# libav/libav

Measured on AMD Instinct MI355X. Metric: macroblocks_per_s, higher is better.
Workload: dtype u8

## Files before the change

include/mi355_h264_frame.h:

```cpp
#ifndef MI355_H264_FRAME_H
#define MI355_H264_FRAME_H

#include <stddef.h>
#include <stdint.h>

#ifdef __cplusplus
extern "C" {
#endif

#define MI355_MB_INTRA4x4    0x00000001u
#define MI355_MB_INTRA16x16  0x00000002u
#define MI355_MB_INTRA_PCM   0x00000004u
#define MI355_MB_16x16       0x00000008u
#define MI355_MB_16x8        0x00000010u
#define MI355_MB_8x16        0x00000020u
#define MI355_MB_8x8         0x00000040u
#define MI355_MB_P0L0        0x00001000u
#define MI355_MB_P1L0        0x00002000u
#define MI355_MB_P0L1        0x00004000u
#define MI355_MB_P1L1        0x00008000u
#define MI355_MB_8x8DCT      0x01000000u
#define MI355_MB_INTRA       (MI355_MB_INTRA4x4 | MI355_MB_INTRA16x16 | MI355_MB_INTRA_PCM)

#define MI355_MBF_LEFT_EDGE  0x01
#define MI355_MBF_TOP_EDGE   0x02
#define MI355_MBF_NO_DEBLOCK 0x04
#define MI355_MBF_WEIGHTED   0x08
#define MI355_MBF_BYPASS     0x10
#define MI355_MBF_BYPASS_PRED 0x20
#define MI355_MBF_BYPASS_X264OLD 0x40
#define MI355_MBF_FILTER_OWN_SLICE 0x80

#define MI355_SUB_8x8  0
#define MI355_SUB_8x4  1
#define MI355_SUB_4x8  2
#define MI355_SUB_4x4  3
#define MI355_SUB_L0   0x10
#define MI355_SUB_L1   0x20

#define MI355_NNZ_LUMA(i)   (i)
#define MI355_NNZ_CB(j)     (16 + (j))
#define MI355_NNZ_CR(j)     (20 + (j))
#define MI355_NNZ_LUMA_DC   24
#define MI355_NNZ_CB_DC     25
#define MI355_NNZ_CR_DC     26

typedef struct mi355_h264_mb {
    uint32_t mb_type;
    uint32_t nnz_mask;
    uint16_t cbp;
    int8_t   qp;
    uint8_t  flags;
    int8_t   slice_alpha_c0_offset;
    int8_t   slice_beta_offset;
    uint8_t  intra16x16_pred_mode;
    uint8_t  chroma_pred_mode;
    uint16_t topleft_samples_available;
    uint16_t topright_samples_available;
    uint8_t  sub_mb_type[4];
    int8_t   ref_idx[2][4];
    uint32_t dc_qmul[3];
    uint8_t  slice_id;
    uint8_t  intra_level;
    uint8_t  qpc[2];
    union {
        int8_t intra4x4_pred_mode[16];
        struct {
            uint8_t ref_pic[2][4];
            int8_t  chroma_dy[2][4];
        } inter;
    } u;
} mi355_h264_mb;

#define MI355_H264_COEFS_PER_MB 384
static inline int mi355_luma_dc_slot(int k)
{
    static const uint8_t col[4] = { 0, 2, 8, 10 }, row[4] = { 0, 1, 4, 5 };
    return 16 * (col[k >> 2] + row[k & 3]);
}


#define MI355_H264_MAX_REFS 16
#define MI355_H264_MAX_SLOTS 32

typedef struct mi355_h264_slice {
    uint8_t use_weight;
    uint8_t use_weight_chroma;
    uint8_t luma_log2_weight_denom;
    uint8_t chroma_log2_weight_denom;
    uint8_t list_count;
    uint8_t reserved[3];
    uint8_t ref_slot[2][MI355_H264_MAX_REFS];
    int16_t luma_weight[MI355_H264_MAX_REFS][2][2];
    int16_t chroma_weight[MI355_H264_MAX_REFS][2][2][2];
    int16_t implicit_weight[MI355_H264_MAX_REFS][MI355_H264_MAX_REFS];
    uint8_t chroma_qp_table[2][52];
    int16_t implicit_weight_field[2][2 * MI355_H264_MAX_REFS][2 * MI355_H264_MAX_REFS];
} mi355_h264_slice;

typedef struct mi355_h264_frame {
    int32_t mb_width, mb_height;
    uint8_t *dst[3];
    int32_t dst_stride[2];
    uint8_t *recon[3];
    int32_t recon_stride[2];
    const uint8_t *ref[MI355_H264_MAX_SLOTS][3];
    const mi355_h264_mb *mb;
    const int16_t *mv[2];
    const int16_t *coef;
    const mi355_h264_slice *slices;
    int32_t nslices;
    int32_t max_intra_level;
    const uint32_t *intra_list;
    const int32_t *intra_level_start;
    int32_t max_level_width;
    int32_t field_picture;
    int32_t surface_layout;
    int32_t flags;
} mi355_h264_frame;
#define MI355_FRAME_NO_INTER 1
#define MI355_FRAME_MBAFF    2

#define MI355_SURFACE_LINEAR 0
#define MI355_SURFACE_TILED  1
#define MI355_LAYOUTS_LINEAR 1
#define MI355_LAYOUTS_TILED  2
#define MI355_TILE_LUMA_BYTES   256
#define MI355_TILE_CHROMA_BYTES 128

typedef struct mi355_surface_job {
    uint8_t *lin[3];
    uint8_t *tiled[2];
    int32_t lin_stride[2];
    int32_t tiled_stride[2];
    int32_t mb_width, mb_height;
    int32_t to_tiled;
    int32_t reserved0;
} mi355_surface_job;
int mi355_h264_surface_convert_dev(const mi355_surface_job *jobs, int n, int max_mb_width, int max_mb_height, void *stream);

int mi355_h264_decode_frames(const mi355_h264_frame *frames, int nframes, void *stream);

int mi355_h264_decode_frames_dev(const mi355_h264_frame *d_frames, int nframes,
                                 int max_mb_width, int max_mb_height, int max_intra_level,
                                 int max_level_width, void *stream);

int mi355_h264_decode_frames_levels_dev(const mi355_h264_frame *d_frames, int nframes,
                                        int max_mb_width, int max_mb_height, int max_intra_level,
                                        const int32_t *level_widths, void *stream);

int mi355_h264_decode_frames_layouts_dev(const mi355_h264_frame *d_frames, int nframes,
                                         int max_mb_width, int max_mb_height, int max_intra_level,
                                         const int32_t *level_widths, int layouts, void *stream);

int mi355_h264_decode_frames_wide_dev(const mi355_h264_frame *d_frames, int nframes, int max_mb_width, int max_mb_height,
                                      int max_intra_level, const int32_t *level_widths, int bit_depth, int chroma_format_idc,
                                      int passes, void *stream);

int mi355_h264_recon_intra_levels_dev(const mi355_h264_frame *d_frames, int nframes, int max_intra_level, const int32_t *level_widths, void *stream);
int mi355_h264_recon_intra_all_dev(const mi355_h264_frame *d_frames, int nframes, int max_mb_width, int max_mb_height, int max_intra_level, const int32_t *level_widths, void *stream);
int mi355_h264_recon_intra_plan(int max_mb_width, int max_mb_height, int max_intra_level, const int32_t *level_widths, int pinned, int *single, long long *per_picture);
int mi355_h264_recon_inter_dev(const mi355_h264_frame *d_frames, int nframes, int max_mb_width, int max_mb_height, void *stream);
int mi355_h264_recon_inter_layouts_dev(const mi355_h264_frame *d_frames, int nframes, int max_mb_width, int max_mb_height, int layouts, void *stream);
int mi355_h264_recon_run_plan(int nframes, int max_mb_width, int max_mb_height, int forced, int *run, int *runs_row);
int mi355_h264_recon_inter_run_dev(const mi355_h264_frame *d_frames, int nframes, int max_mb_width, int max_mb_height, int run, void *stream);
int mi355_h264_recon_inter_sparse_dev(const mi355_h264_frame *d_frames, int nframes, int max_mb_width, int max_mb_height, void *stream);
int mi355_h264_recon_intra_dev(const mi355_h264_frame *d_frames, int nframes, int max_intra_level, int max_level_width, void *stream);
int mi355_h264_deblock_dev(const mi355_h264_frame *d_frames, int nframes, int max_mb_width, int max_mb_height, void *stream);
int mi355_h264_deblock_layouts_dev(const mi355_h264_frame *d_frames, int nframes, int max_mb_width, int max_mb_height, int layouts, void *stream);

typedef struct mi355_h264_deblock_plan_info {
    int32_t tiled_waves;
    int32_t linear_bands;
    int32_t skip_tiled;
    int32_t linear_launches;
} mi355_h264_deblock_plan_info;
int mi355_h264_deblock_plan(int nframes, int max_mb_width, int max_mb_height, int layouts, int cus, mi355_h264_deblock_plan_info *plan);
int mi355_h264_deblock_form_dev(const mi355_h264_frame *d_frames, int nframes, int max_mb_width, int max_mb_height, int layouts,
                                int tiled_waves, int linear_bands, void *stream);

int mi355_h264_intra_schedule(mi355_h264_mb *mb, int mb_width, int mb_height,
                              uint32_t *list, int32_t *level_start, int *max_level_width);

int mi355_h264_intra_schedule_mbaff(mi355_h264_mb *mb, int mb_width, int mb_height,
                                    uint32_t *list, int32_t *level_start, int *max_level_width);

void *mi355_malloc(size_t bytes);
void  mi355_free(void *dptr);
int   mi355_memcpy_h2d(void *dst, const void *src, size_t bytes);
int   mi355_memcpy_d2h(void *dst, const void *src, size_t bytes);
int   mi355_memcpy_d2d(void *dst, const void *src, size_t bytes);
int   mi355_sync(void *stream);
void  mi355_prefer_blocking_sync(int on);
void *mi355_host_alloc(size_t bytes);
void  mi355_host_free(void *p);
int   mi355_memcpy_h2d_async(void *dst, const void *src, size_t bytes, void *stream);
int   mi355_memcpy_d2h_async(void *dst, const void *src, size_t bytes, void *stream);
int   mi355_memcpy2d_d2h_async(void *dst, size_t dst_pitch, const void *src, size_t src_pitch, size_t width_bytes, size_t rows, void *stream);
int   mi355_memcpy2d_d2d_async(void *dst, size_t dst_pitch, const void *src, size_t src_pitch, size_t width_bytes, size_t rows, void *stream);
int   mi355_event_sync(void *event);
typedef struct mi355_copy_job {
    const void *src;
    void *dst;
    uint64_t bytes;
} mi355_copy_job;
int   mi355_copy_batch_dev(const mi355_copy_job *jobs, int n, size_t max_bytes, void *stream);
typedef struct mi355_h264_pipelines mi355_h264_pipelines;
mi355_h264_pipelines *mi355_h264_pipelines_create(int shares, int turns);
void mi355_h264_pipelines_destroy(mi355_h264_pipelines *p);
int  mi355_h264_pipelines_decode_dev(mi355_h264_pipelines *p, const mi355_h264_frame *d_frames, int nframes, int max_mb_width, int max_mb_height,
                                     int max_intra_level, const int32_t *level_widths, int layouts);
int  mi355_h264_pipelines_sync(mi355_h264_pipelines *p);
int  mi355_h264_pipelines_share(const mi355_h264_pipelines *p, int nframes, int share, int *first, int *count);
void mi355_h264_pipelines_timing(mi355_h264_pipelines *p, int on);
void mi355_h264_pipelines_join(mi355_h264_pipelines *p, int mode);
int  mi355_h264_pipelines_collect(mi355_h264_pipelines *p, double sums[3], int *launches);

void *mi355_stream_create(void);
void  mi355_stream_destroy(void *stream);
int   mi355_stream_wait_event(void *stream, void *event);
void *mi355_event_create(void);
void  mi355_event_destroy(void *event);
int   mi355_event_record(void *event, void *stream);
int   mi355_event_query(void *event);
float mi355_event_elapsed_ms(void *start, void *end);

#ifdef __cplusplus
}
#endif
#endif
```

libav_amd/csrc/h264_deblock.hip:

```cpp
#include <cstdlib>
#include <vector>
#include "h264_deblock_dev.h"

using namespace mi355;

namespace {

#ifdef MI355_PROF
__device__ unsigned long long g_prof[16];
#define PROF_MARK(i) do { const unsigned long long now_ = __builtin_readcyclecounter(); prof_acc[i] += now_ - prof_t; prof_t = now_; } while (0)
#else
#define PROF_MARK(i) do { } while (0)
#endif

#ifndef MI355_DCH_LOG
#define MI355_DCH_LOG 2
#endif
constexpr int DCH_LOG = MI355_DCH_LOG, DCH = 1 << DCH_LOG;
#ifndef MI355_DPAD
#define MI355_DPAD 8
#endif
constexpr int DY_PITCH = 16 * DCH + MI355_DPAD;
constexpr int DC_PITCH = 8 * DCH + MI355_DPAD;
constexpr int DIO_ROWS = 16 / DCH;
// ... 543 lines not shown
        if (lane < 52) {
            s.t_alpha[lane] = k_alpha[lane]; s.t_beta[lane] = k_beta[lane];
            s.t_tc0[lane] = ((uint32_t)k_tc0[lane][0] << 8) | ((uint32_t)k_tc0[lane][1] << 16) | ((uint32_t)k_tc0[lane][2] << 24);
        }
        if (lane < 16) {
            const int seg = l >> 2, edge = l & 3, qe = edge == 0 ? 3 : edge - 1;
            const bool outer = edge == 0;
            uint32_t *r = s.role[l];
            r[0] = 1u << blk_index(edge, seg); r[1] = 1u << blk_index(qe, seg); r[2] = 8u * ((edge >> 1) + 2 * (seg >> 1)); r[3] = 8u * ((qe >> 1) + 2 * (seg >> 1));
            r[4] = 1u << blk_index(seg, edge); r[5] = 1u << blk_index(seg, qe); r[6] = 8u * ((seg >> 1) + 2 * (edge >> 1)); r[7] = 8u * ((seg >> 1) + 2 * (qe >> 1));
            r[8] = (uint32_t)(4 * (edge + 4 * seg));
            r[9] = (uint32_t)(outer ? 4 * (3 + 4 * seg) - 64 : 4 * (edge - 1 + 4 * seg));
            r[10] = (uint32_t)(4 * (seg + 4 * edge));
            r[11] = (uint32_t)(outer ? 4 * (seg + 12) - 64 * W : 4 * (seg + 4 * (edge - 1)));
        }
    }
    if (NW == 1) MI355_WAVE_SYNC(); else MI355_WG_BARRIER_LDS();

    uint8_t *const lds = reinterpret_cast<uint8_t *>(&s);
    constexpr uint32_t OY = (uint32_t)offsetof(Deblock3Lds, y), OC = (uint32_t)offsetof(Deblock3Lds, c), OA = (uint32_t)offsetof(Deblock3Lds, above);
    uint32_t k_g2, k_rec, k_topd, k_dy, k_dc, k_gc2, k_da, k_sab, k_sc, k_sd, k_se, k_la, k_lc, k_ld, k_rv, k_cv, k_flags;
    uint32_t k_pl, k_pc, k_hy, k_ha, k_hc, k_hca;
    enum { KF_ROW = 1, KF_TOP = 2, KF_BOTTOM = 4, KF_LO = 8, KF_G0 = 16, KF_ROW0 = 32, KF_CSRC_SHIFT = 8, KF_EDGE8_SHIFT = 16 };
    constexpr uint32_t OP = (uint32_t)offsetof(Deblock3Lds, parm), PB = (uint32_t)sizeof(uint32_t[4][9][2]);
    {
        const int lane = lane_id(), g = lane >> 4, l = lane & 15, ga = (g - 1) & 3;
        const int mb_y = 4 * band + g, mb_yc = mb_y < H ? mb_y : H - 1;
        const bool row_ok = mb_y < H, has_t = row_ok && mb_y > 0, bottom = row_ok && (g == 3 || mb_y == H - 1), lo = l < 8;
        k_flags = (row_ok ? KF_ROW : 0) | (has_t ? KF_TOP : 0) | (bottom ? KF_BOTTOM : 0) | (lo ? KF_LO : 0) | (g == 0 ? KF_G0 : 0) | (mb_yc == 0 ? KF_ROW0 : 0);
        k_flags |= (uint32_t)(4 * ((lane & ~15) | (((l & 7) >> 1) << 2))) << KF_CSRC_SHIFT;
        k_flags |= (uint32_t)(8 * (l & 3)) << KF_EDGE8_SHIFT;
        k_g2 = (uint32_t)(2 * g);
        k_rec = (uint32_t)(64 * mb_yc * W);
        k_topd = mb_yc > 0 ? 64u * (uint32_t)W : 0u;
        k_dy = (uint32_t)(mb_yc * rs + 16 * (l ^ g));
        {
            const int gc = (lane >> 3) & 3, q = lane & 7, yc = 4 * band + gc < H ? 4 * band + gc : H - 1;
            k_dc = (uint32_t)(yc * rcs + 16 * (q ^ gc));
            k_gc2 = (uint32_t)(2 * gc);
        }
        k_da = (lane & 8) ? (uint32_t)(ya * dcs + 16 * ((lane & 7) ^ 3)) : (uint32_t)(ya * ds + 128 + 16 * ((lane & 7) ^ 3));
        k_sab = lo ? (uint32_t)(mb_y * ds - (2 * g + 1) * 256 + 16 * l) : (uint32_t)((mb_y - 1) * ds - 2 * g * 256 + 16 * l);
        k_sc = (uint32_t)((mb_y - 1) * dcs - 2 * g * 128 + 8 * l);
        k_sd = (uint32_t)(mb_y * ds - (2 * g + 1) * 256 + 128 + 8 * l);
        k_se = (uint32_t)(mb_y * dcs - (2 * g + 1) * 128 + 8 * l);
        k_rv = (uint32_t)(256 * g + 16 * (l ^ g));
        k_cv = (uint32_t)(128 * g + 16 * ((l >> 1) ^ g) + 8 * (l & 1));
        k_la = lo ? k_rv : (uint32_t)(g ? 256 * ga + 128 + 16 * ((l - 8) ^ ga) : 16 * ((l - 8) ^ 3));
        k_lc = (uint32_t)(g ? 128 * ga + 16 * ((l >> 1) ^ ga) + 8 * (l & 1) : 128 + 16 * ((l >> 1) ^ 3) + 8 * (l & 1));
        k_ld = (uint32_t)(256 * g + 16 * ((8 + (l >> 1)) ^ g) + 8 * (l & 1));
        k_pl = OP + (uint32_t)(72 * g);
        k_pc = k_pl + (uint32_t)(24 + 24 * (l >> 3));
        k_hy = (uint32_t)(256 * g + 16 * g + l);
        k_ha = (uint32_t)(g ? 256 * ga + 128 + 64 + 16 * ga + l : 64 + 16 * 3 + l);
        k_hc = (uint32_t)(128 * g + 16 * g + 64 * (l >> 3) + (l & 7));
        k_hca = (uint32_t)(g ? 128 * ga + 16 * (ga ^ 3) + 64 * (l >> 3) + (l & 7) : 128 + 64 * (l >> 3) + (l & 7));
        static_assert((OY & 63) == 0 && (OC & 63) == 0 && (OA & 63) == 0, "bits 4 and 5 of a column's address are the swizzle's alone");
    }
    auto kf = [&](uint32_t bit) { return (k_flags & bit) != 0; };
    auto prefetch = [&](Pre &p, int t1) {
        const int l = lane_id() & 15;
        const bool outer = (l & 3) == 0;
        const int xc = med3i(t1 - (int)k_g2, 0, W - 1);
        const uint32_t roff = k_rec + ((uint32_t)xc << 6), toff = roff - k_topd;
        mb_prefetch<TWO_LISTS>(p, rec_base, mv_base0, mv_base1, roff, toff, &s.role[l][8], outer, xc, k_flags & KF_ROW0);
    };
    auto dma_issue = [&](int t1) {
        const int lane = lane_id();
        lds_dma16<false>(recon_y0 + (k_dy + ((uint32_t)med3i(t1 - (int)k_g2, 0, W - 1) << 8)), &s.y[t1 & 3][0][0]);
        if (lane < 32) lds_dma16<false>(recon_c0 + (k_dc + ((uint32_t)med3i(t1 - (int)k_gc2, 0, W - 1) << 7)), &s.c[t1 & 3][0][0]);
        if (top_band && lane < 16) {
            const int xa = t1 < W ? t1 : W - 1;
            const uint8_t *src = (lane & 8) ? dst_c0 + (k_da + ((uint32_t)xa << 7)) : dst_y0 + (k_da + ((uint32_t)xa << 8));
            lds_dma16<true>(src, &s.above[t1 & 1][0]);
        }
        MI355_ISSUE_FENCE();
    };
    uint32_t seen = 0;
    auto await_above = [&](int x0) {
        if (!top_band) return;
        const uint32_t need = (uint32_t)(x0 + 1 < W ? x0 + 1 : W);
        if (seen >= need) return;
        for (;;) {
            seen = (uint32_t)uniform((int)agent_load_u32(mi355_global_v(prog_above)));
            if (seen >= need) break;
            wave_nap();
        }
        MI355_ISSUE_FENCE();
    };
    auto stores = [&](int ts) {
        const uint32_t u1y = OY + 1024u * (uint32_t)((ts - 1) & 3), u2y = OY + 1024u * (uint32_t)((ts - 2) & 3), ua = OA + 256u * (uint32_t)(ts & 1);
        const uint32_t u1c = OC + 512u * (uint32_t)((ts - 1) & 3), u2c = OC + 512u * (uint32_t)((ts - 2) & 3);
        const uint32_t xhi = (uint32_t)ts - k_g2, xlo = xhi - 1u;
        const bool in_lo = xlo < (uint32_t)W, in_hi = xhi < (uint32_t)W;
        const bool lo = kf(KF_LO), g0 = kf(KF_G0);
        const bool ok = lo ? (kf(KF_ROW) && in_lo) : (kf(KF_TOP) && in_hi);
        const uint4 v = lds16(lds + (k_la + (lo ? u1y : (g0 ? ua : u2y))));
        if (ok) st16(dst_y0 + (k_sab + ((uint32_t)ts << 8)), v, true);
        const uint2 vc = *reinterpret_cast<const uint2 *>(lds + (k_lc + (g0 ? ua : u2c)));
        if (kf(KF_TOP) && in_hi) st8(dst_c0 + (k_sc + ((uint32_t)ts << 7)), vc, true);
        const uint2 by = *reinterpret_cast<const uint2 *>(lds + (k_ld + u1y)), bc = *reinterpret_cast<const uint2 *>(lds + (k_cv + u1c));
        if (!hand && kf(KF_BOTTOM) && in_lo) {
            st8(dst_y0 + (k_sd + ((uint32_t)ts << 8)), by, true);
            st8(dst_c0 + (k_se + ((uint32_t)ts << 7)), bc, true);
        }
        MI355_WAVE_SYNC();
    };

    auto hand_down = [&](int t) {
        const uint32_t u1y = OY + 1024u * (uint32_t)((t - 1) & 3), u1c = OC + 512u * (uint32_t)((t - 1) & 3);
        const uint32_t xlo = (uint32_t)t - k_g2 - 1u;
        const uint2 by = *reinterpret_cast<const uint2 *>(lds + (k_ld + u1y)), bc = *reinterpret_cast<const uint2 *>(lds + (k_cv + u1c));
        if (kf(KF_BOTTOM) && xlo < (uint32_t)W) {
            agent_store8(dst_y0 + (k_sd + ((uint32_t)t << 8)), by, true);
            agent_store8(dst_c0 + (k_se + ((uint32_t)t << 7)), bc, true);
        }
    };
    Pre pre = {}, pre_next = {};
    MbInfo hl = {};
    auto strengths = [&](int t, int pb, uint32_t &bsw0, uint32_t &bsw1, uint32_t &bsc0, uint32_t &bsc1) {
        const int l = lane_id() & 15;
        const int mb_x = t - (int)k_g2;
        const bool has_t = kf(KF_TOP), valid = kf(KF_ROW) && (uint32_t)mb_x < (uint32_t)W;
        const bool outer = (l & 3) == 0, odd = (l & 1) != 0;
        const MbInfo &h = pre.h, &ht = pre.ht;
        const mi355_u32x4 ra = *reinterpret_cast<const mi355_u32x4 *>(&s.role[l][0]), rb = *reinterpret_cast<const mi355_u32x4 *>(&s.role[l][4]);
        const BsRole r0{ ra[0], ra[1], ra[2], ra[3] }, r1{ rb[0], rb[1], rb[2], rb[3] };
        const bool filter = valid && !(h.flags() & MI355_MBF_NO_DEBLOCK);
        const bool have_left = filter && mb_x > 0 && (h.flags() & MI355_MBF_LEFT_EDGE), have_top = filter && has_t && (h.flags() & MI355_MBF_TOP_EDGE);
        const uint32_t b0 = bs_role(h, hl, outer, odd, filter && (!outer || have_left), r0, pre.p0, pre.q0, two_lists, mv_far, 4u);
        const uint32_t b1 = bs_role(h, ht, outer, odd, filter && (!outer || have_top), r1, pre.p1, pre.q1, two_lists, mv_far, field ? 3u : 4u);
        const uint32_t edge8 = k_flags >> KF_EDGE8_SHIFT;
        bsw0 = quad_or(b0 << edge8); bsw1 = quad_or(b1 << edge8);
        const uint32_t csrc4 = (k_flags >> KF_CSRC_SHIFT) & 0xFFu;
        bsc0 = lane_gather4(bsw0, csrc4); bsc1 = lane_gather4(bsw1, csrc4);
        const int comp = l < 3 ? 0 : (l < 6 ? 1 : 2), kind = l - 3 * comp;
        const int kindc = kind > 2 ? 2 : kind;
        const MbInfo &nb = kindc == 1 ? hl : ht;
        int qa = comp ? h.qpc(comp - 1) : h.qp();
        int qb = comp ? nb.qpc(comp - 1) : nb.qp();
        if (comp && kindc && nb.slice_id() != h.slice_id() && (kindc == 1 ? have_left : have_top)) {
            int v = mi355_global(fr.slices)[h.slice_id()].chroma_qp_table[comp - 1][nb.qp()];
            MI355_PIN(v);
            qb = v;
        }
        const int qp = kindc ? (qa + qb + 1) >> 1 : qa;
        const int ia = clip3(qp + h.alpha_off(), 0, 51), ib = clip3(qp + h.beta_off(), 0, 51);
        const uint32_t w0 = (uint32_t)s.t_alpha[ia] | ((uint32_t)s.t_beta[ib] << 8);
        const uint32_t w1 = s.t_tc0[ia] + (comp ? 0x01010100u : 0u);
        if (l < 9) *reinterpret_cast<mi355_u32x2 *>(lds + (k_pl + PB * (uint32_t)pb + 8u * (uint32_t)l)) = mi355_u32x2{ w0, w1 };
        hl = h;
    };
    auto edges_v = [&](int t, int pb, uint32_t bsw0, uint32_t bsc0) {
        {
            const uint32_t *pl = reinterpret_cast<const uint32_t *>(lds + (k_pl + PB * (uint32_t)pb)), *pc = reinterpret_cast<const uint32_t *>(lds + (k_pc + PB * (uint32_t)pb));
            const uint32_t ab_i = pl[0], tr_i = pl[1], ab_l = pl[2], tr_l = pl[3];
            const uint32_t cab_i = pc[0], ctr_i = pc[1], cab_l = pc[2], ctr_l = pc[3];
            const uint32_t tci0 = byte_perm(0, tr_i, bsw0 & 0x03030303u), tcl0 = byte_perm(0, tr_l, bsw0 & 3u);
            const uint32_t cci0 = byte_perm(0, ctr_i, bsc0 & 0x03030303u), ccl0 = byte_perm(0, ctr_l, bsc0 & 3u);
            uint8_t *rowp = lds + (k_rv + OY + 1024u * (uint32_t)(t & 3)), *leftp = lds + (k_rv + OY + 12u + 1024u * (uint32_t)((t - 1) & 3));
            uint8_t *crowp = lds + (k_cv + OC + 512u * (uint32_t)(t & 3)), *cleftp = lds + (k_cv + OC + 4u + 512u * (uint32_t)((t - 1) & 3));
            vertical_edges<true>(rowp, leftp, crowp, cleftp, bsw0, bsc0, ab_l, ab_i, tcl0, tci0, cab_l, cab_i, ccl0, cci0);
        }
    };
    auto edges_h = [&](int t, int pb, uint32_t bsw1, uint32_t bsc1) {
        {
            const uint32_t *pl = reinterpret_cast<const uint32_t *>(lds + (k_pl + PB * (uint32_t)pb)), *pc = reinterpret_cast<const uint32_t *>(lds + (k_pc + PB * (uint32_t)pb));
            const uint32_t ab_i = pl[0], tr_i = pl[1], ab_t = pl[4], tr_t = pl[5];
            const uint32_t cab_i = pc[0], ctr_i = pc[1], cab_t = pc[4], ctr_t = pc[5];
            const uint32_t tci1 = byte_perm(0, tr_i, bsw1 & 0x03030303u), tct1 = byte_perm(0, tr_t, bsw1 & 3u);
            const uint32_t cci1 = byte_perm(0, ctr_i, bsc1 & 0x03030303u), cct1 = byte_perm(0, ctr_t, bsc1 & 3u);
            const bool g0 = kf(KF_G0);
            const uint32_t ua = OA + 256u * (uint32_t)(t & 1);
            const uint32_t yb = k_hy + (OY + 1024u * (uint32_t)(t & 3)), cb = k_hc + (OC + 512u * (uint32_t)(t & 3));
            const uint32_t ab = k_ha + (g0 ? ua : OY + 1024u * (uint32_t)((t - 2) & 3)), cab = k_hca + (g0 ? ua : OC + 512u * (uint32_t)((t - 2) & 3));
            uint8_t *const Y0 = lds + yb, *const Y1 = lds + (yb ^ 16u), *const Y2 = lds + (yb ^ 32u), *const Y3 = lds + (yb ^ 48u);
            uint8_t *const A0 = lds + ab, *const A1 = lds + (ab ^ 16u), *const A2 = lds + (ab ^ 32u), *const A3 = lds + (ab ^ 48u);
            uint8_t *const C0 = lds + cb, *const C1 = lds + (cb ^ 16u), *const C2 = lds + (cb ^ 32u), *const CA3 = lds + cab;
#define YJ(j) ((j) == 0 ? Y0 : ((j) == 1 ? Y1 : ((j) == 2 ? Y2 : Y3)))
#define AJ(j) ((j) == 0 ? A0 : ((j) == 1 ? A1 : ((j) == 2 ? A2 : A3)))
#define YR(r) YJ((r) & 3)[64 * ((r) >> 2)]
#define AR(r) AJ((r) & 3)[0]
#define CR(r) (((r) >> 1) == 0 ? C0 : (((r) >> 1) == 1 ? C1 : C2))[8 * ((r) & 1)]
#define CAR(r) CA3[8 * ((r) & 1)]
            int y0 = AR(12), y1 = AR(13), y2 = AR(14), y3 = AR(15);
            int y4 = YR(0), y5 = YR(1), y6 = YR(2), y7 = YR(3), y8 = YR(4), y9 = YR(5), y10 = YR(6), y11 = YR(7);
            int y12 = YR(8), y13 = YR(9), y14 = YR(10), y15 = YR(11), y16 = YR(12), y17 = YR(13), y18 = YR(14);
            int u0 = CAR(6), u1 = CAR(7), u2 = CR(0), u3 = CR(1), u4 = CR(2), u5 = CR(3), u6 = CR(4), u7 = CR(5);
            const int e0 = luma_line<true, true>(y0, y1, y2, y3, y4, y5, y6, y7, byte_of(bsw1, 0), ab_alpha(ab_t), ab_beta(ab_t), byte_of(tct1, 0));
            if (e0) {
                if (e0 == 2) { AR(13) = (uint8_t)y1; YR(2) = (uint8_t)y6; }
                AR(14) = (uint8_t)y2; AR(15) = (uint8_t)y3; YR(0) = (uint8_t)y4; YR(1) = (uint8_t)y5;
            }
            if (luma_line<false, true>(y4, y5, y6, y7, y8, y9, y10, y11, byte_of(bsw1, 1), ab_alpha(ab_i), ab_beta(ab_i), byte_of(tci1, 1))) {
                YR(2) = (uint8_t)y6; YR(3) = (uint8_t)y7; YR(4) = (uint8_t)y8; YR(5) = (uint8_t)y9;
            }
            if (luma_line<false, true>(y8, y9, y10, y11, y12, y13, y14, y15, byte_of(bsw1, 2), ab_alpha(ab_i), ab_beta(ab_i), byte_of(tci1, 2))) {
                YR(6) = (uint8_t)y10; YR(7) = (uint8_t)y11; YR(8) = (uint8_t)y12; YR(9) = (uint8_t)y13;
            }
            int y19 = 0;
            if (luma_line<false, true>(y12, y13, y14, y15, y16, y17, y18, y19, byte_of(bsw1, 3), ab_alpha(ab_i), ab_beta(ab_i), byte_of(tci1, 3))) {
                YR(10) = (uint8_t)y14; YR(11) = (uint8_t)y15; YR(12) = (uint8_t)y16; YR(13) = (uint8_t)y17;
            }
            if (chroma_line<true>(u0, u1, u2, u3, byte_of(bsc1, 0), ab_alpha(cab_t), ab_beta(cab_t), byte_of(cct1, 0))) {
                CAR(7) = (uint8_t)u1; CR(0) = (uint8_t)u2;
            }
            if (chroma_line<true>(u4, u5, u6, u7, byte_of(bsc1, 2), ab_alpha(cab_i), ab_beta(cab_i), byte_of(cci1, 2))) {
                CR(3) = (uint8_t)u5; CR(4) = (uint8_t)u6;
            }
#undef YJ
#undef AJ
#undef YR
#undef AR
#undef CR
#undef CAR
        }
    };
    if constexpr (NW == 1) {
        await_above(0);
        dma_issue(0);
        prefetch(pre, 0);
        hl = pre.h;
#pragma nounroll
        for (int t = 0; t < nsteps; t++) {
            agent_drain_stores();
            if (hand && t >= 8) {
                const int done = t - 7 < W ? t - 7 : W;
                if (lane_id() == 0) agent_store_u32(mi355_global_v(prog_self), (uint32_t)done);
            }
            MI355_WAVE_SYNC();
            if (t > 0) stores(t - 1);
            await_above(t + 1);
            dma_issue(t + 1);
            uint32_t bsw0, bsw1, bsc0, bsc1;
            strengths(t, 0, bsw0, bsw1, bsc0, bsc1);
            prefetch(pre, t + 1);
            MI355_WAVE_SYNC();
            edges_v(t, 0, bsw0, bsc0);
            MI355_WAVE_SYNC();
            if (hand) hand_down(t);
            edges_h(t, 0, bsw1, bsc1);
        }
        agent_drain_stores();
        MI355_WAVE_SYNC();
        stores(nsteps - 1);
    } else {
        if (srv_wave) {
            await_above(0);
            dma_issue(0);
            prefetch(pre, 0);
            hl = pre.h;
            uint32_t b[4];
            strengths(0, 0, b[0], b[1], b[2], b[3]);
            *reinterpret_cast<mi355_u32x4 *>(mail->bs[0][lane_id()]) = mi355_u32x4{ b[0], b[1], b[2], b[3] };
            prefetch(pre_next, 1);
        }
#pragma nounroll
        for (int t = 0; t < nsteps; t++) {
            agent_drain_stores();
            if (edge_wave && hand && t >= 8) {
                const int done = t - 7 < W ? t - 7 : W;
                if (lane_id() == 0) agent_store_u32(mi355_global_v(prog_self), (uint32_t)done);
            }
            MI355_WG_BARRIER_LDS();
            if (edge_wave) {
                const mi355_u32x4 b = *reinterpret_cast<const mi355_u32x4 *>(mail->bs[t & 1][lane_id()]);
                edges_v(t, t & 1, b[0], b[2]);
                MI355_WAVE_SYNC();
                if (hand) hand_down(t);
                edges_h(t, t & 1, b[1], b[3]);
            } else {
                pre = pre_next;
                prefetch(pre_next, t + 2);
                if (t > 0) stores(t - 1);
                await_above(t + 1);
                dma_issue(t + 1);
                uint32_t b[4];
                strengths(t + 1, (t + 1) & 1, b[0], b[1], b[2], b[3]);
                *reinterpret_cast<mi355_u32x4 *>(mail->bs[(t + 1) & 1][lane_id()]) = mi355_u32x4{ b[0], b[1], b[2], b[3] };
            }
            MI355_WG_BARRIER_LDS();
        }
        if (!srv_wave) {
            if (hand) {
                agent_drain_stores();
                if (lane_id() == 0) agent_store_u32(mi355_global_v(prog_self), (uint32_t)W);
            }
            return;
        }
        agent_drain_stores();
        stores(nsteps - 1);
        return;
    }
    if (hand) {
        agent_drain_stores();
        if (lane_id() == 0) agent_store_u32(mi355_global_v(prog_self), (uint32_t)W);
    }
}

#ifdef MI355_DB3_WAVES
__attribute__((amdgpu_waves_per_eu(MI355_DB3_WAVES, MI355_DB3_WAVES)))
#endif
__global__ void __launch_bounds__(64)
k_deblock_tiled(const mi355_h264_frame *__restrict__ frames, int nframes, int nbands, uint32_t *sync)
{
    __shared__ Deblock3Lds s;
    uint32_t tk = 0;
    if (lane_id() == 0) tk = atomicAdd(mi355_global(sync), 1u);
    tk = (uint32_t)lane_value((int)tk, 0);
    const int band = (int)(tk / (uint32_t)nframes), pic = (int)(tk - (uint32_t)band * (uint32_t)nframes);
    if (band >= nbands) return;
    const mi355_h264_frame &fr = frames[pic];
    if (4 * band >= uniform(fr.mb_height) || uniform(fr.surface_layout) != MI355_SURFACE_TILED) return;
    uint32_t *prog = mi355_global(sync) + 16 + (size_t)pic * (size_t)nbands;
    if (mi355_global(fr.mv[1]) != nullptr) deblock3_band<true, 1>(s, nullptr, fr, band, prog, 0);
    else deblock3_band<false, 1>(s, nullptr, fr, band, prog, 0);
}
__global__ void __launch_bounds__(128)
k_deblock_tiled2(const mi355_h264_frame *__restrict__ frames, int nframes, int nbands, uint32_t *sync)
{
    __shared__ Deblock3Lds s;
    __shared__ Deblock3Mail mail;
    __shared__ uint32_t ticket;
    if (threadIdx.x == 0) ticket = atomicAdd(mi355_global(sync), 1u);
    __syncthreads();
    const uint32_t tk = (uint32_t)uniform((int)ticket);
    const int wave = uniform((int)(threadIdx.x >> 6));
    const int band = (int)(tk / (uint32_t)nframes), pic = (int)(tk - (uint32_t)band * (uint32_t)nframes);
    if (band >= nbands) return;
    const mi355_h264_frame &fr = frames[pic];
    if (4 * band >= uniform(fr.mb_height) || uniform(fr.surface_layout) != MI355_SURFACE_TILED) return;
    uint32_t *prog = mi355_global(sync) + 16 + (size_t)pic * (size_t)nbands;
    if (mi355_global(fr.mv[1]) != nullptr) deblock3_band<true, 2>(s, &mail, fr, band, prog, wave);
    else deblock3_band<false, 2>(s, &mail, fr, band, prog, wave);
}

}

#ifdef MI355_PROF
extern "C" void mi355_debug_prof(unsigned long long *out, int reset)
{
    unsigned long long z[16] = {};
    MI355_CHECK(hipDeviceSynchronize());
    MI355_CHECK(hipMemcpyFromSymbol(out, HIP_SYMBOL(g_prof), sizeof(z)));
    if (reset) MI355_CHECK(hipMemcpyToSymbol(HIP_SYMBOL(g_prof), z, sizeof(z)));
}
#endif

namespace {
struct SyncBuf {
    int device;
    hipStream_t stream;
    uint32_t *dev;
    size_t words;
};
}
static std::vector<SyncBuf> &sync_pool() { static thread_local std::vector<SyncBuf> pool; return pool; }
uint32_t *mi355::sync_words(hipStream_t st, size_t words)
{
    std::vector<SyncBuf> &pool = sync_pool();
    const int device = mi355::current_device();
    SyncBuf *b = nullptr;
    for (SyncBuf &e : pool)
        if (e.device == device && e.stream == st) { b = &e; break; }
    if (!b) {
        pool.push_back(SyncBuf{ device, st, nullptr, 0 });
        b = &pool.back();
    }
    if (b->dev && b->words >= words) return b->dev;
    if (b->dev) (void)hipFree(b->dev);
    b->dev = nullptr; b->words = 0;
    size_t n = 4096;
    while (n < words) n *= 2;
    if (hipMalloc(reinterpret_cast<void **>(&b->dev), n * sizeof(uint32_t)) != hipSuccess) { b->dev = nullptr; return nullptr; }
    b->words = n;
    return b->dev;
}
void mi355::sync_words_release(hipStream_t st)
{
    std::vector<SyncBuf> &pool = sync_pool();
    const int device = mi355::current_device();
    for (size_t i = 0; i < pool.size(); i++)
        if (pool[i].device == device && pool[i].stream == st) {
            if (pool[i].dev) (void)hipFree(pool[i].dev);
            pool.erase(pool.begin() + (long)i);
            return;
        }
}

namespace {
int deblock_form_pin()
{
    static const int force = std::getenv("MI355_DEBLOCK_FORM") ? std::atoi(std::getenv("MI355_DEBLOCK_FORM")) : 0;
    return force;
}
int deblock_waves_pin()
{
    static const int pin = std::getenv("MI355_DEBLOCK_WAVES") ? std::atoi(std::getenv("MI355_DEBLOCK_WAVES")) : 0;
    return pin;
}
int device_cus()
{
    static int cus = 0;
    if (!cus) {
        hipDeviceProp_t prop;
        int dev = 0;
        cus = hipGetDevice(&dev) == hipSuccess && hipGetDeviceProperties(&prop, dev) == hipSuccess && prop.multiProcessorCount > 0 ? prop.multiProcessorCount : 256;
    }
    return cus;
}
bool linear_form(int kw) { return kw == 1 || kw == 2 || kw == 3 || kw == 4 || kw == 6; }

mi355_h264_deblock_plan_info deblock_plan(int nframes, int max_mb_width, int max_mb_height, int layouts, int cus)
{
    const int nbands = (max_mb_height + 3) / 4, nsteps = max_mb_width + 6;
    const int force = deblock_form_pin();
    mi355_h264_deblock_plan_info p{ 0, 0, 0, 0 };
    const bool tiled_launch = (layouts & MI355_LAYOUTS_TILED) && force == 0;
    if (tiled_launch) {
        const int pin = deblock_waves_pin();
        const long long simds = 4LL * cus;
        p.tiled_waves = pin == 2 || (pin != 1 && (long long)nframes * nbands < 2LL * simds) ? 2 : 1;
        if (!(layouts & MI355_LAYOUTS_LINEAR)) return p;
    }
    int best = 1;
    double best_cost = 0;
    const int forms[5] = { 1, 2, 3, 4, 6 };
    for (int i = 0; i < 5; i++) {
        const int kw = forms[i];
        const long resident = (long)cus * (DEBLOCK_WAVES_PER_CU / kw);
        const double rounds = (double)((nframes + resident - 1) / resident);
        const double cost = rounds * ((nbands + kw - 1) / kw) * (nsteps + DEBLOCK_LAG * (kw - 1)) * (kw > 1 ? 1.25 : 1.0);
        if (i == 0 || cost < best_cost) { best = kw; best_cost = cost; }
    }
    if (linear_form(force)) best = force;
    p.linear_bands = best;
    p.skip_tiled = tiled_launch ? 1 : 0;
    p.linear_launches = (nbands + best - 1) / best;
    return p;
}

int deblock_launch(const mi355_h264_frame *d_frames, int nframes, int nbands, const mi355_h264_deblock_plan_info &p, hipStream_t st)
{
    if (p.tiled_waves) {
        if ((long long)nframes * nbands > 0x7FFFFFFFLL) return -3;
        const size_t words = 16 + (size_t)nframes * (size_t)nbands;
        uint32_t *sync = mi355::sync_words(st, words);
        if (!sync) return -4;
        MI355_TRY(hipMemsetAsync(sync, 0, words * sizeof(uint32_t), st), -4);
        if (p.tiled_waves == 2) hipLaunchKernelGGL(k_deblock_tiled2, dim3((unsigned)(nframes * nbands)), dim3(128), 0, st, d_frames, nframes, nbands, sync);
        else hipLaunchKernelGGL(k_deblock_tiled, dim3((unsigned)(nframes * nbands)), dim3(64), 0, st, d_frames, nframes, nbands, sync);
    }
    for (int band = 0; p.linear_bands && band < nbands; band += p.linear_bands) {
        const dim3 grid((unsigned)nframes);
        switch (p.linear_bands) {
        case 2: hipLaunchKernelGGL(k_deblock_bands<2>, grid, dim3(128), 0, st, d_frames, band, p.skip_tiled); break;
        case 3: hipLaunchKernelGGL(k_deblock_bands<3>, grid, dim3(192), 0, st, d_frames, band, p.skip_tiled); break;
        case 4: hipLaunchKernelGGL(k_deblock_bands<4>, grid, dim3(256), 0, st, d_frames, band, p.skip_tiled); break;
        case 6: hipLaunchKernelGGL(k_deblock_bands<6>, grid, dim3(384), 0, st, d_frames, band, p.skip_tiled); break;
        default: hipLaunchKernelGGL(k_deblock, grid, dim3(64), 0, st, d_frames, band, p.skip_tiled); break;
        }
    }
    return hipGetLastError() == hipSuccess ? 0 : -2;
}
}

extern "C" int mi355_h264_deblock_dev(const mi355_h264_frame *d_frames, int nframes, int max_mb_width, int max_mb_height, void *stream)
{
    return mi355_h264_deblock_layouts_dev(d_frames, nframes, max_mb_width, max_mb_height, MI355_LAYOUTS_LINEAR | MI355_LAYOUTS_TILED, stream);
}

static int deblock_args(const mi355_h264_frame *d_frames, int nframes, int max_mb_width, int max_mb_height, int layouts)
{
    if (!mi355::bind() || !d_frames || nframes <= 0 || !(layouts & (MI355_LAYOUTS_LINEAR | MI355_LAYOUTS_TILED))) return 0;
    const int nbands = (max_mb_height + 3) / 4;
    return nbands <= 0 || max_mb_width <= 0 ? 0 : nbands;
}

extern "C" int mi355_h264_deblock_layouts_dev(const mi355_h264_frame *d_frames, int nframes, int max_mb_width, int max_mb_height, int layouts, void *stream)
{
    const int nbands = deblock_args(d_frames, nframes, max_mb_width, max_mb_height, layouts);
    if (!nbands) return -1;
    return deblock_launch(d_frames, nframes, nbands, deblock_plan(nframes, max_mb_width, max_mb_height, layouts, device_cus()), (hipStream_t)stream);
}

extern "C" int mi355_h264_deblock_plan(int nframes, int max_mb_width, int max_mb_height, int layouts, int cus, mi355_h264_deblock_plan_info *plan)
{
    if (!plan || nframes <= 0 || max_mb_width <= 0 || max_mb_height <= 0 || cus < 0 || !(layouts & (MI355_LAYOUTS_LINEAR | MI355_LAYOUTS_TILED))) return -1;
    if (cus == 0) {
        if (!mi355::bind()) return -1;
        cus = device_cus();
    }
    *plan = deblock_plan(nframes, max_mb_width, max_mb_height, layouts, cus);
    return 0;
}

extern "C" int mi355_h264_deblock_form_dev(const mi355_h264_frame *d_frames, int nframes, int max_mb_width, int max_mb_height, int layouts, int tiled_waves,
                                           int linear_bands, void *stream)
{
    const int nbands = deblock_args(d_frames, nframes, max_mb_width, max_mb_height, layouts);
    if (!nbands) return -1;
    if (tiled_waves < 0 || tiled_waves > 2 || (linear_bands != 0 && !linear_form(linear_bands))) return -1;
    if ((layouts & MI355_LAYOUTS_LINEAR) && !linear_bands) return -1;
    if ((layouts & MI355_LAYOUTS_TILED) && !tiled_waves && !linear_bands) return -1;
    if (tiled_waves && !(layouts & MI355_LAYOUTS_TILED)) return -1;
    const mi355_h264_deblock_plan_info p{ tiled_waves, linear_bands, tiled_waves ? 1 : 0, linear_bands ? (nbands + linear_bands - 1) / linear_bands : 0 };
    return deblock_launch(d_frames, nframes, nbands, p, (hipStream_t)stream);
}
```

libav_amd/csrc/h264_pipelines.hip:

```cpp
#include "mi355_rt.h"
#include "mi355_h264_frame.h"

#include <vector>

struct mi355_h264_pipelines {
    int shares = 0, turns = 1, device = -1;
    bool started = false;
    bool started_done = false;
    std::vector<hipStream_t> stream;
    std::vector<hipEvent_t> turn;
    std::vector<hipEvent_t> done;
    int join = 1;
    const void *last_frames = nullptr;
    int last_nframes = -1;
    std::vector<hipEvent_t> pool;
    std::vector<hipEvent_t> spare;
    bool timing = false;
};

extern "C" mi355_h264_pipelines *mi355_h264_pipelines_create(int shares, int turns)
{
    if (shares < 1 || shares > 16 || !mi355::bind()) return nullptr;
    mi355_h264_pipelines *p = new mi355_h264_pipelines;
    p->shares = shares; p->turns = turns != 0; p->device = mi355::current_device();
    for (int i = 0; i < shares; i++) {
        hipStream_t st = nullptr;
        hipEvent_t ev = nullptr, dn = nullptr;
        if (hipStreamCreateWithFlags(&st, hipStreamNonBlocking) != hipSuccess || hipEventCreateWithFlags(&ev, hipEventDisableTiming) != hipSuccess ||
            hipEventCreateWithFlags(&dn, hipEventDisableTiming) != hipSuccess) {
            if (st) (void)hipStreamDestroy(st);
            if (ev) (void)hipEventDestroy(ev);
            for (hipStream_t s : p->stream) (void)hipStreamDestroy(s);
            for (hipEvent_t e : p->turn) (void)hipEventDestroy(e);
            for (hipEvent_t e : p->done) (void)hipEventDestroy(e);
            delete p;
            return nullptr;
        }
        p->stream.push_back(st); p->turn.push_back(ev); p->done.push_back(dn);
    }
    return p;
}

extern "C" int mi355_h264_pipelines_sync(mi355_h264_pipelines *p)
{
    if (!p) return -1;
    int rc = 0;
    for (hipStream_t st : p->stream) if (hipStreamSynchronize(st) != hipSuccess) rc = -2;
    return rc ? rc : mi355::fault_after_wait();
}

extern "C" void mi355_h264_pipelines_destroy(mi355_h264_pipelines *p)
{
    if (!p) return;
    (void)mi355_h264_pipelines_sync(p);
    for (hipStream_t st : p->stream) { mi355::sync_words_release(st); (void)hipStreamDestroy(st); }
    for (hipEvent_t e : p->turn) (void)hipEventDestroy(e);
    for (hipEvent_t e : p->done) (void)hipEventDestroy(e);
    for (hipEvent_t e : p->pool) (void)hipEventDestroy(e);
    for (hipEvent_t e : p->spare) (void)hipEventDestroy(e);
    delete p;
}

extern "C" void mi355_h264_pipelines_timing(mi355_h264_pipelines *p, int on) { if (p) p->timing = on != 0; }
extern "C" void mi355_h264_pipelines_join(mi355_h264_pipelines *p, int mode) { if (p && mode >= 0 && mode <= 2) p->join = mode; }

extern "C" int mi355_h264_pipelines_share(const mi355_h264_pipelines *p, int nframes, int share, int *first, int *count)
{
    if (!p || share < 0 || share >= p->shares || nframes < 0) return -1;
    const int q = nframes / p->shares, r = nframes % p->shares;
    if (first) *first = share * q + (share < r ? share : r);
    if (count) *count = q + (share < r ? 1 : 0);
    return 0;
}

extern "C" int mi355_h264_pipelines_decode_dev(mi355_h264_pipelines *p, const mi355_h264_frame *d_frames, int nframes, int max_mb_width, int max_mb_height,
                                               int max_intra_level, const int32_t *level_widths, int layouts)
{
    if (!p || !d_frames || nframes <= 0 || !mi355::bind()) return -1;
    const bool joined = p->started_done && (p->join == 2 || (p->join == 1 && (d_frames != p->last_frames || nframes != p->last_nframes)));
    const size_t pool0 = p->pool.size();
    auto fail = [&](int rc) -> int {
        while (p->pool.size() > pool0) { p->spare.push_back(p->pool.back()); p->pool.pop_back(); }
        return rc;
    };
    auto stamp = [&](hipStream_t st) -> int {
        if (!p->timing) return 0;
        hipEvent_t e = nullptr;
        if (!p->spare.empty()) { e = p->spare.back(); p->spare.pop_back(); }
        else if (hipEventCreateWithFlags(&e, hipEventDefault) != hipSuccess) return -4;
        if (hipEventRecord(e, st) != hipSuccess) { p->spare.push_back(e); return -4; }
        p->pool.push_back(e);
        return 0;
    };
#define PIPE_TRY(call) do { if ((call) != hipSuccess) return fail(-4); } while (0)
    if (joined)
        for (int i = 0; i < p->shares; i++)
            for (int k = 0; k < p->shares; k++)
                if (k != i) PIPE_TRY(hipStreamWaitEvent(p->stream[(size_t)i], p->done[(size_t)k], 0));
    for (int i = 0; i < p->shares; i++) {
        int first = 0, count = 0;
        (void)mi355_h264_pipelines_share(p, nframes, i, &first, &count);
        hipStream_t st = p->stream[(size_t)i];
        if (count <= 0) {
            if (p->turns && p->started && p->shares > 1) PIPE_TRY(hipStreamWaitEvent(st, p->turn[(size_t)((i + p->shares - 1) % p->shares)], 0));
            if (p->turns) { PIPE_TRY(hipEventRecord(p->turn[(size_t)i], st)); p->started = true; }
            if (p->timing) for (int k = 0; k < 4; k++) { const int rc = stamp(st); if (rc) return fail(rc); }
            PIPE_TRY(hipEventRecord(p->done[(size_t)i], st));
            continue;
        }
        const mi355_h264_frame *d = d_frames + first;
        if (p->turns && p->shares > 1 && (i > 0 || p->started)) PIPE_TRY(hipStreamWaitEvent(st, p->turn[(size_t)((i + p->shares - 1) % p->shares)], 0));
        int rc = stamp(st);
        if (rc) return fail(rc);
        rc = mi355_h264_recon_inter_layouts_dev(d, count, max_mb_width, max_mb_height, layouts, st);
        if (rc) return fail(rc);
        if (p->turns) { PIPE_TRY(hipEventRecord(p->turn[(size_t)i], st)); p->started = true; }
        if ((rc = stamp(st))) return fail(rc);
        rc = mi355_h264_recon_intra_all_dev(d, count, max_mb_width, max_mb_height, max_intra_level, level_widths, st);
        if (rc) return fail(rc);
        if ((rc = stamp(st))) return fail(rc);
        rc = mi355_h264_deblock_layouts_dev(d, count, max_mb_width, max_mb_height, layouts, st);
        if (rc) return fail(rc);
        if ((rc = stamp(st))) return fail(rc);
        PIPE_TRY(hipEventRecord(p->done[(size_t)i], st));
    }
#undef PIPE_TRY
    p->started_done = true;
    p->last_frames = d_frames; p->last_nframes = nframes;
    return 0;
}

extern "C" int mi355_h264_pipelines_collect(mi355_h264_pipelines *p, double sums[3], int *launches)
{
    if (!p) return -1;
    const int rc = mi355_h264_pipelines_sync(p);
    if (rc) return rc;
    for (size_t i = 0; i + 3 < p->pool.size(); i += 4) {
        for (int k = 0; k < 3; k++) {
            float ms = 0.f;
            if (hipEventElapsedTime(&ms, p->pool[i + (size_t)k], p->pool[i + (size_t)k + 1]) != hipSuccess) return -4;
            if (sums) sums[k] += ms;
        }
        if (launches) ++*launches;
    }
    p->spare.insert(p->spare.end(), p->pool.begin(), p->pool.end());
    p->pool.clear();
    return 0;
}
```

Before: 1.500 billion.

## Run tiled deblock as persistent resident waves when pipelines share the GPU

```diff
diff --git a/include/mi355_h264_frame.h b/include/mi355_h264_frame.h
--- a/include/mi355_h264_frame.h
+++ b/include/mi355_h264_frame.h
@@ -168,6 +168,9 @@
 int mi355_h264_recon_intra_dev(const mi355_h264_frame *d_frames, int nframes, int max_intra_level, int max_level_width, void *stream);
 int mi355_h264_deblock_dev(const mi355_h264_frame *d_frames, int nframes, int max_mb_width, int max_mb_height, void *stream);
 int mi355_h264_deblock_layouts_dev(const mi355_h264_frame *d_frames, int nframes, int max_mb_width, int max_mb_height, int layouts, void *stream);
+int mi355_h264_deblock_resident_dev(const mi355_h264_frame *d_frames, int nframes, int max_mb_width, int max_mb_height, int layouts,
+                                    int resident_waves, void *stream);
+int mi355_h264_deblock_resident(int nframes, int max_mb_width, int max_mb_height, int layouts, int cus, int shares, int *resident_waves);
 
 typedef struct mi355_h264_deblock_plan_info {
     int32_t tiled_waves;
diff --git a/libav_amd/csrc/h264_deblock.hip b/libav_amd/csrc/h264_deblock.hip
--- a/libav_amd/csrc/h264_deblock.hip
+++ b/libav_amd/csrc/h264_deblock.hip
@@ -869,19 +869,25 @@
 __attribute__((amdgpu_waves_per_eu(MI355_DB3_WAVES, MI355_DB3_WAVES)))
 #endif
 __global__ void __launch_bounds__(64)
-k_deblock_tiled(const mi355_h264_frame *__restrict__ frames, int nframes, int nbands, uint32_t *sync)
+k_deblock_tiled(const mi355_h264_frame *__restrict__ frames, int nframes, int nbands, uint32_t *sync, int turns)
 {
     __shared__ Deblock3Lds s;
-    uint32_t tk = 0;
-    if (lane_id() == 0) tk = atomicAdd(mi355_global(sync), 1u);
-    tk = (uint32_t)lane_value((int)tk, 0);
-    const int band = (int)(tk / (uint32_t)nframes), pic = (int)(tk - (uint32_t)band * (uint32_t)nframes);
-    if (band >= nbands) return;
-    const mi355_h264_frame &fr = frames[pic];
-    if (4 * band >= uniform(fr.mb_height) || uniform(fr.surface_layout) != MI355_SURFACE_TILED) return;
-    uint32_t *prog = mi355_global(sync) + 16 + (size_t)pic * (size_t)nbands;
-    if (mi355_global(fr.mv[1]) != nullptr) deblock3_band<true, 1>(s, nullptr, fr, band, prog, 0);
-    else deblock3_band<false, 1>(s, nullptr, fr, band, prog, 0);
+    const uint32_t ntickets = (uint32_t)nframes * (uint32_t)nbands;
+    do {
+        uint32_t tk = 0;
+        if (lane_id() == 0) tk = atomicAdd(mi355_global(sync), 1u);
+        tk = (uint32_t)lane_value((int)tk, 0);
+        if (tk >= ntickets) return;
+        const int band = (int)(tk / (uint32_t)nframes), pic = (int)(tk - (uint32_t)band * (uint32_t)nframes);
+        const mi355_h264_frame &fr = frames[pic];
+        if (4 * band >= uniform(fr.mb_height) || uniform(fr.surface_layout) != MI355_SURFACE_TILED) continue;
+        uint32_t *prog = mi355_global(sync) + 16 + (size_t)pic * (size_t)nbands;
+        if (mi355_global(fr.mv[1]) != nullptr) deblock3_band<true, 1>(s, nullptr, fr, band, prog, 0);
+        else deblock3_band<false, 1>(s, nullptr, fr, band, prog, 0);
+        if (!turns) return;
+        agent_drain_stores();
+        MI355_WAVE_SYNC();
+    } while (turns);
 }
 __global__ void __launch_bounds__(128)
 k_deblock_tiled2(const mi355_h264_frame *__restrict__ frames, int nframes, int nbands, uint32_t *sync)
@@ -966,6 +972,11 @@
     static const int pin = std::getenv("MI355_DEBLOCK_WAVES") ? std::atoi(std::getenv("MI355_DEBLOCK_WAVES")) : 0;
     return pin;
 }
+int deblock_resident_pin()
+{
+    static const int pin = std::getenv("MI355_DEBLOCK_RESIDENT") ? std::atoi(std::getenv("MI355_DEBLOCK_RESIDENT")) : 0;
+    return pin;
+}
 int device_cus()
 {
     static int cus = 0;
@@ -1007,7 +1018,16 @@
     return p;
 }
 
-int deblock_launch(const mi355_h264_frame *d_frames, int nframes, int nbands, const mi355_h264_deblock_plan_info &p, hipStream_t st)
+constexpr int DEBLOCK_RESIDENT_HALVES = 3;
+long long deblock_resident_rule(long long simds, long long tickets, int shares)
+{
+    long long n = tickets;
+    if (shares > 1 && DEBLOCK_RESIDENT_HALVES > 0) n = (simds * DEBLOCK_RESIDENT_HALVES + 1) / 2;
+    if (deblock_resident_pin() > 0) n = deblock_resident_pin();
+    return n < 1 ? 1 : (n < tickets ? n : tickets);
+}
+
+int deblock_launch(const mi355_h264_frame *d_frames, int nframes, int nbands, const mi355_h264_deblock_plan_info &p, hipStream_t st, long long resident = 0)
 {
     if (p.tiled_waves) {
         if ((long long)nframes * nbands > 0x7FFFFFFFLL) return -3;
@@ -1016,7 +1036,11 @@
         if (!sync) return -4;
         MI355_TRY(hipMemsetAsync(sync, 0, words * sizeof(uint32_t), st), -4);
         if (p.tiled_waves == 2) hipLaunchKernelGGL(k_deblock_tiled2, dim3((unsigned)(nframes * nbands)), dim3(128), 0, st, d_frames, nframes, nbands, sync);
-        else hipLaunchKernelGGL(k_deblock_tiled, dim3((unsigned)(nframes * nbands)), dim3(64), 0, st, d_frames, nframes, nbands, sync);
+        else {
+            const long long tickets = (long long)nframes * nbands;
+            const bool turns = resident > 0 && resident < tickets;
+            hipLaunchKernelGGL(k_deblock_tiled, dim3((unsigned)(turns ? resident : tickets)), dim3(64), 0, st, d_frames, nframes, nbands, sync, turns ? 1 : 0);
+        }
     }
     for (int band = 0; p.linear_bands && band < nbands; band += p.linear_bands) {
         const dim3 grid((unsigned)nframes);
@@ -1051,6 +1075,29 @@
     return deblock_launch(d_frames, nframes, nbands, deblock_plan(nframes, max_mb_width, max_mb_height, layouts, device_cus()), (hipStream_t)stream);
 }
 
+extern "C" int mi355_h264_deblock_resident_dev(const mi355_h264_frame *d_frames, int nframes, int max_mb_width, int max_mb_height, int layouts, int resident_waves, void *stream)
+{
+    const int nbands = deblock_args(d_frames, nframes, max_mb_width, max_mb_height, layouts);
+    if (!nbands || resident_waves < 0) return -1;
+    mi355_h264_deblock_plan_info p = deblock_plan(nframes, max_mb_width, max_mb_height, layouts, device_cus());
+    if (resident_waves && p.tiled_waves == 2) p.tiled_waves = 1;
+    const long long resident = resident_waves ? resident_waves : deblock_resident_rule(4LL * device_cus(), (long long)nframes * nbands, 2);
+    return deblock_launch(d_frames, nframes, nbands, p, (hipStream_t)stream, resident);
+}
+
+extern "C" int mi355_h264_deblock_resident(int nframes, int max_mb_width, int max_mb_height, int layouts, int cus, int shares, int *resident_waves)
+{
+    if (!resident_waves || nframes <= 0 || max_mb_width <= 0 || max_mb_height <= 0 || cus < 0 || shares < 1 || !(layouts & (MI355_LAYOUTS_LINEAR | MI355_LAYOUTS_TILED))) return -1;
+    if (cus == 0) {
+        if (!mi355::bind()) return -1;
+        cus = device_cus();
+    }
+    const long long tickets = (long long)nframes * ((max_mb_height + 3) / 4);
+    if (tickets > 0x7FFFFFFFLL) return -1;
+    *resident_waves = deblock_plan(nframes, max_mb_width, max_mb_height, layouts, cus).tiled_waves == 1 ? (int)deblock_resident_rule(4LL * cus, tickets, shares) : 0;
+    return 0;
+}
+
 extern "C" int mi355_h264_deblock_plan(int nframes, int max_mb_width, int max_mb_height, int layouts, int cus, mi355_h264_deblock_plan_info *plan)
 {
     if (!plan || nframes <= 0 || max_mb_width <= 0 || max_mb_height <= 0 || cus < 0 || !(layouts & (MI355_LAYOUTS_LINEAR | MI355_LAYOUTS_TILED))) return -1;
diff --git a/libav_amd/csrc/h264_pipelines.hip b/libav_amd/csrc/h264_pipelines.hip
--- a/libav_amd/csrc/h264_pipelines.hip
+++ b/libav_amd/csrc/h264_pipelines.hip
@@ -119,7 +119,10 @@
         rc = mi355_h264_recon_intra_all_dev(d, count, max_mb_width, max_mb_height, max_intra_level, level_widths, st);
         if (rc) return fail(rc);
         if ((rc = stamp(st))) return fail(rc);
-        rc = mi355_h264_deblock_layouts_dev(d, count, max_mb_width, max_mb_height, layouts, st);
+        int resident = 0;
+        if (mi355_h264_deblock_resident(count, max_mb_width, max_mb_height, layouts, 0, p->shares, &resident)) return fail(-1);
+        rc = resident ? mi355_h264_deblock_resident_dev(d, count, max_mb_width, max_mb_height, layouts, resident, st)
+                      : mi355_h264_deblock_layouts_dev(d, count, max_mb_width, max_mb_height, layouts, st);
         if (rc) return fail(rc);
         if ((rc = stamp(st))) return fail(rc);
         PIPE_TRY(hipEventRecord(p->done[(size_t)i], st));
```

Result: faster. 1.538 billion, median of 6 (+2.5%).
